# ksadov/FREUD

Measured on AMD Instinct MI355X. Metric: SAE train activations/sec (d=384 dict 8x), higher is better.
Workload: dtype bf16; 1 GPU; Whisper-tiny d=384 dict 8x (n=3072) L1 SAE train step, M=65536 rows/GPU/step, RAdam+cosine, x bfloat16 resident in HBM (BASELINE configs[1]); rows_per_gpu=65536, d_model=384, n_dict=3072, parallelism=dp1, dp=none

## Files before the change

freud_amd/csrc/engine.hip:

```cpp
#include <hip/hip_runtime.h>
#include <math.h>
#include <stdarg.h>
#include <stdio.h>
#include <string.h>

#include <algorithm>
#include <utility>
#include <vector>

#include "../../include/freud_sae.h"
#include "l1_kernels.h"
#include "gemm256.h"
#include "gemm256s.h"
#include "gemm256_fp8.h"
#include "l1_fp8.h"
#include "dp_kernels.h"
#include "p2p_exchange.h"
#include <rccl/rccl.h>
#include <mutex>
#include <unistd.h>

static thread_local bool g_force_gemm128 = false;
static thread_local bool g_no_stream = false;
static thread_local int g_device = 0;
// ... 1398 lines not shown
  g2.nbm = g.nbm / 2;
  g2.nbn = g.nbn / 2;
  hipLaunchKernelGGL(kerns, dim3(G2_PERSIST_STATIC), dim3(512), G2S_LDS_BYTES, s, g2, epi);
  HIP_TRY(hipGetLastError());
  return SAE_OK;
}

template <int AM, int BM_, class Epi>
static int launch_gemm(const GemmArgs& g, const Epi& epi, hipStream_t s) {
  if constexpr (epi_stream<Epi>::value && AM == OP_ROW && BM_ == OP_ROW) {
    if (gemm_streams<AM, BM_, Epi>(g)) return launch_gemm_stream(g, epi, s);
  }
  if (!g_force_gemm128 && g.nbm % 2 == 0 && g.nbn % 2 == 0) {
    auto kern256 = gemm256_bf16_kernel<AM, BM_, Epi>;
    constexpr bool a3 = epi_deep_a_ring<Epi>::value;
    constexpr int lds256 = a3 ? G2_A3_LDS_BYTES : (epi_rounds_first<Epi>::value && G2_BF16_LDS_BYTES > G2_LDS_BYTES) ? G2_BF16_LDS_BYTES : G2_LDS_BYTES;
    static_assert(G2_A3_LDS_BYTES >= G2_BF16_LDS_BYTES && G2_A3_LDS_BYTES >= G2_LDS_BYTES, "the epilogues reuse the ring's LDS");
    LDS_ATTR(kern256, lds256, g_device);
    GemmArgs g2 = g;
    g2.nbm = g.nbm / 2;
    g2.nbn = g.nbn / 2;
    const int grid_max = (g.dyn && g.grid_cover > 0) ? g.grid_cover
                         : g2.tail_tiles > 0    ? g2.nbm * g2.nbn + g2.tail_tiles * (g2.tail_pieces - 1)
                                                : g2.nbm * g2.nbn * g2.splits;
    const int grid_est = (((g.grid_hint + 3) / 4 + 7) / 8) * 8;
    if (G2_PERSIST_STATIC > 0 && !g.dyn && g2.splits == 1 && g2.tail_tiles == 0 && grid_max >= 4 * G2_PERSIST_STATIC) {
      auto kernp = gemm256_bf16_kernel<AM, BM_, Epi, true>;
      LDS_ATTR(kernp, lds256, g_device);
      hipLaunchKernelGGL(kernp, dim3(G2_PERSIST_STATIC), dim3(512), lds256, s, g2, epi);
    } else if (g.dyn && g.grid_hint > 0 && grid_est < grid_max) {
      auto kernp = gemm256_bf16_kernel<AM, BM_, Epi, true>;
      LDS_ATTR(kernp, lds256, g_device);
      hipLaunchKernelGGL(kernp, dim3(grid_est < 256 ? 256 : grid_est), dim3(512), lds256, s, g2, epi);
    } else {
      hipLaunchKernelGGL(kern256, dim3(grid_max), dim3(512), lds256, s, g2, epi);
    }
    HIP_TRY(hipGetLastError());
    return SAE_OK;
  }
  auto kern = gemm_bf16_kernel<AM, BM_, Epi>;
  LDS_ATTR(kern, GEMM_LDS_BYTES, g_device);
  const int grid = (g.dyn && g.grid_cover > 0) ? g.grid_cover : g.nbm * g.nbn * g.splits;
  hipLaunchKernelGGL(kern, dim3(grid), dim3(256), GEMM_LDS_BYTES, s, g, epi);
  HIP_TRY(hipGetLastError());
  return SAE_OK;
}

template <class Epi>
static bool gemm8_streams(const Gemm8Args& g) {
  if constexpr (!epi_stream<Epi>::value) return false;
  return !g_no_stream && g.ktiles >= 2 && g.lda == g.ldb && g.nbm * g.nbn >= 4 * G2_PERSIST_STATIC;
}

template <class Epi>
static int launch_gemm8(const Gemm8Args& g, const Epi& epi, hipStream_t s) {
  if constexpr (epi_stream<Epi>::value) {
    if (gemm8_streams<Epi>(g)) {
      auto kerns = gemm256s_fp8_kernel<Epi>;
      LDS_ATTR(kerns, G2S_LDS_BYTES, g_device);
      hipLaunchKernelGGL(kerns, dim3(G2_PERSIST_STATIC), dim3(512), G2S_LDS_BYTES, s, g, epi);
      HIP_TRY(hipGetLastError());
      return SAE_OK;
    }
  }
  auto kern = gemm256_fp8_kernel<Epi>;
  constexpr int lds = g8_lds_bytes<Epi>();
  LDS_ATTR(kern, lds, g_device);
  hipLaunchKernelGGL(kern, dim3(g.nbm * g.nbn), dim3(512), lds, s, g, epi);
  HIP_TRY(hipGetLastError());
  return SAE_OK;
}

static void prep_weights_l1(sae_ctx* c, hipStream_t s) {
  const int d_p = c->d_p, n_p = c->n_p;
  float* W = c->P;
  if (c->wn_pending && !c->wn_fwd_seen) {
    c->wn_fwd_seen = true;
  } else {
    settle_weights(c, s);
    if (!c->cn_valid) hipLaunchKernelGGL(colnorm_partial_kernel, dim3(n_p / 128, d_p / 32), dim3(256), 0, s, W, c->cn_part, n_p);
    c->cn_valid = false;
    hipLaunchKernelGGL(normalize_cast_kernel, dim3(n_p / 64, d_p / 64), dim3(256), 0, s, W, c->cn_part, d_p / 32, c->Wb,
                       c->Wt, d_p, n_p);
  }
}

template <typename T>
static int launch_prep_x(sae_ctx* c, const T* x, int64_t M, int64_t Mp, hipStream_t s) {
  const int d = c->d, d_p = c->d_p;
  const int grid = grid_for(Mp * (d_p / 8), 2048);
  if (d % 8 == 0 && (reinterpret_cast<uintptr_t>(x) & 15) == 0)
    hipLaunchKernelGGL((prep_x_kernel<T, true>), dim3(grid), dim3(256), 0, s, x, c->xb, c->masked, M, d, Mp, d_p);
  else
    hipLaunchKernelGGL((prep_x_kernel<T, false>), dim3(grid), dim3(256), 0, s, x, c->xb, c->masked, M, d, Mp, d_p);
  return grid;
}

static GemmArgs enc_gemm_args(const sae_ctx* c, const bf16_t* xb, int64_t Mp) {
  GemmArgs g{};
  g.A0 = xb; g.B0 = c->Wt; g.lda = c->d_p; g.ldb = c->d_p;
  g.nbm = (int)(Mp / 128); g.nbn = c->n_p / 128; g.ktiles0 = g.ktiles = c->d_p / 64; g.splits = 1;
  return g;
}

template <typename T>
static auto launch_encoder(sae_ctx* c, const GemmArgs& g, int64_t M, hipStream_t s) {
  EpiEnc e{};
  e.c = c->c; e.bias = c->P + c->nW; e.l1_part = c->l1_part; e.M = M; e.n_p = c->n_p; e.nbn = g.nbn;
  if (gemm_streams<OP_ROW, OP_ROW, EpiEnc>(g)) HIP_TRY(hipMemsetAsync(c->l1_part, 0, (size_t)g.nbm * g.nbn * 4, s));
  ev_begin(c, KID_ENC_FWD, s);
  const int rc = launch_gemm<OP_ROW, OP_ROW>(g, e, s);
  ev_end(c, KID_ENC_FWD, s);
  return rc;
}

template <typename T> static constexpr bool x_dtype_is_bf16() { return false; }
template <> constexpr bool x_dtype_is_bf16<bf16_t>() { return true; }

template <typename T>
static int forward_impl(sae_ctx* c, const T* x, int64_t M, int64_t Mp, hipStream_t s, bool need_backward) {
  const int d = c->d, d_p = c->d_p, n_p = c->n_p;
  const float alpha = (float)c->cfg.recon_alpha;
  float* W = c->P;
  float* b = c->P + c->nW;

  ev_begin(c, KID_PREP_W, s);
  prep_weights_l1(c, s);
  if (c->fp8) hipLaunchKernelGGL(fp8_cast_w_kernel, dim3(n_p / 64, d_p / 64), dim3(256), 0, s, W, c->W8, c->W8t, d_p, n_p);
  ev_end(c, KID_PREP_W, s);

  ev_begin(c, KID_PREP_X, s);
  const bool alias_x = c->use_fused_fwd && sizeof(T) == 2 && x_dtype_is_bf16<T>() && d == d_p && M == Mp &&
                       (reinterpret_cast<uintptr_t>(x) & 15) == 0;
  c->xb_cur = alias_x ? reinterpret_cast<const bf16_t*>(x) : c->xb;
  if (!alias_x) {
    const int grid = launch_prep_x(c, x, M, Mp, s);
    if (!c->use_fused_fwd) {
      const double* gs = (need_backward && c->dp_world > 0) ? c->stats : nullptr;
      if (gs && c->dist) HIP_TRY(hipStreamWaitEvent(s, c->ev_stats, 0));
      hipLaunchKernelGGL(finalize_count_kernel, dim3(1), dim3(256), 0, s, c->masked, grid, c->scal, M, d, alpha, gs);
    }
  }
  if (c->fp8) {
    const int sgrid = (int)((Mp / 4) < 1024 ? (Mp / 4) : 1024);
    hipLaunchKernelGGL(fp8_x_stats_kernel, dim3(sgrid), dim3(256), 0, s, c->xb, Mp, d_p, c->x8_part);
    hipLaunchKernelGGL(fp8_scales_kernel, dim3(1), dim3(256), 0, s, c->x8_part, sgrid, b, c->n, c->scal8);
    const int64_t n8 = Mp * (d_p / 8);
    hipLaunchKernelGGL(fp8_quant_x_kernel, dim3(grid_for(n8, 2048)), dim3(256), 0, s, c->xb, c->x8, n8, c->scal8);
  }
  ev_end(c, KID_PREP_X, s);

  int rc;
  if (c->use_fused_fwd) {
    const int lds = FF_LDS_BYTES;
    FwdFusedArgs a{};
    a.xb = c->xb_cur; a.x = x; a.Wt = c->Wt; a.bias = b; a.cnt_part = c->cnt_part; a.c = c->c; a.dxh = c->dxh;
    a.l1_part = c->l1_part; a.sq_part = c->sq_part; a.M = M; a.d = d; a.n_p = n_p; a.ntiles = n_p / FF_BN;
    a.c_rows = c->max_rows_p;
    const int full_wgs = (int)(M / FF_BM), all_wgs = (int)(Mp / FF_BM);
    auto launch = [&](auto kern, int blocks, int block_offset) -> int {
      LDS_ATTR(kern, 160 * 1024, g_device);
      a.block_offset = block_offset;
      hipLaunchKernelGGL(kern, dim3(blocks), dim3(256), lds, s, a);
      return SAE_OK;
    };
    ev_begin(c, KID_FWD_FUSED, s);
    int rcl = SAE_OK;
    if (full_wgs > 0 && c->cfg.debug_flags == 65 && c->fwd_variant == 1) {
      a.stamps = reinterpret_cast<unsigned long long*>(c->dpre);
      rcl = launch(fwd_fused_d384_kernel<T, false, true>, full_wgs, 0);
    } else if (c->fwd_variant == 2) {
      if (full_wgs > 0 && c->cfg.debug_flags == 65) {
        a.stamps = reinterpret_cast<unsigned long long*>(c->dpre);
        rcl = launch(fwd_fused2_d384_kernel<T, false, true>, full_wgs, 0);
      } else if (full_wgs > 0) rcl = launch(fwd_fused2_d384_kernel<T, false>, full_wgs, 0);
      if (!rcl && all_wgs > full_wgs) rcl = launch(fwd_fused2_d384_kernel<T, true>, all_wgs - full_wgs, full_wgs);
      if (rcl) return rcl;
      ev_end(c, KID_FWD_FUSED, s);
      HIP_TRY(hipGetLastError());
      return SAE_OK;
    } else if (full_wgs > 0) {
      rcl = launch(fwd_fused_d384_kernel<T, false, false>, full_wgs, 0);
    }
    if (!rcl && all_wgs > full_wgs) rcl = launch(fwd_fused_d384_kernel<T, true, false>, all_wgs - full_wgs, full_wgs);
    if (rcl) return rcl;
    ev_end(c, KID_FWD_FUSED, s);
    HIP_TRY(hipGetLastError());
    return SAE_OK;
  }
  if (c->fp8) {
    {
      Gemm8Args g{};
      g.A = c->x8; g.B = c->W8t; g.lda = d_p; g.ldb = d_p;
      g.nbm = (int)(Mp / 256); g.nbn = n_p / 256; g.ktiles = d_p / 128;
      EpiEnc8 e{};
      e.c = c->c; e.c8 = c->c8; e.bias = b; e.scal8 = c->scal8; e.l1_part = c->l1_part; e.M = M; e.n_p = n_p; e.nbn = n_p / 128;
      if (gemm8_streams<EpiEnc8>(g)) HIP_TRY(hipMemsetAsync(c->l1_part, 0, (size_t)(Mp / 128) * (n_p / 128) * 4, s));
      ev_begin(c, KID_ENC_FWD, s);
      rc = launch_gemm8(g, e, s);
      ev_end(c, KID_ENC_FWD, s);
      if (rc) return rc;
    }
    {
      Gemm8Args g{};
      g.A = c->c8; g.B = c->W8; g.lda = n_p; g.ldb = n_p;
      g.nbm = (int)(Mp / 256); g.nbn = d_p / 256; g.ktiles = n_p / 128;
      EpiDec<T> e{};
      e.x = x; e.dxh = c->dxh; e.scal = c->scal; e.sq_part = c->sq_part; e.M = M; e.d = d; e.d_p = d_p; e.nbn = d_p / 128;
      e.vec_all = (M == Mp && d == d_p && d % 4 == 0 && (reinterpret_cast<uintptr_t>(x) % (4 * sizeof(T))) == 0) ? 1 : 0;
      e.vscale = c->scal8 + S8_INV_DEC;
      ev_begin(c, KID_DEC_FWD, s);
      rc = launch_gemm8(g, e, s);
      ev_end(c, KID_DEC_FWD, s);
      if (rc) return rc;
    }
    if (need_backward && c->dxhT) {
      hipLaunchKernelGGL(transpose_bf16_kernel, dim3((unsigned)(Mp / 64), d_p / 64), dim3(256), 0, s, c->dxh, c->dxhT, Mp, d_p);
      hipLaunchKernelGGL(transpose_bf16_kernel, dim3((unsigned)(Mp / 64), d_p / 64), dim3(256), 0, s, c->xb_cur, c->xT, Mp, d_p);
      HIP_TRY(hipGetLastError());
    }
    return SAE_OK;
  }
  rc = launch_encoder<T>(c, enc_gemm_args(c, c->xb_cur, Mp), M, s);
  if (rc) return rc;
  {
    GemmArgs g{};
    g.A0 = c->c; g.B0 = c->Wb; g.lda = n_p; g.ldb = n_p;
    g.nbm = (int)(Mp / 128); g.nbn = d_p / 128; g.ktiles0 = g.ktiles = n_p / 64; g.splits = 1;
    g.group_m = 4;
    EpiDec<T> e{};
    e.x = x; e.dxh = c->dxh; e.scal = c->scal; e.sq_part = c->sq_part; e.M = M; e.d = d; e.d_p = d_p; e.nbn = g.nbn;
    e.vec_all = (M == Mp && d == d_p && d % 4 == 0 && (reinterpret_cast<uintptr_t>(x) % (4 * sizeof(T))) == 0) ? 1 : 0;
    ev_begin(c, KID_DEC_FWD, s);
    rc = launch_gemm<OP_ROW, OP_ROW>(g, e, s);
    ev_end(c, KID_DEC_FWD, s);
    if (rc) return rc;
  }
  if (need_backward && c->dxhT) {
    hipLaunchKernelGGL(transpose_bf16_kernel, dim3((unsigned)(Mp / 64), d_p / 64), dim3(256), 0, s, c->dxh, c->dxhT, Mp, d_p);
    hipLaunchKernelGGL(transpose_bf16_kernel, dim3((unsigned)(Mp / 64), d_p / 64), dim3(256), 0, s, c->xb_cur, c->xT, Mp, d_p);
    HIP_TRY(hipGetLastError());
  }
  return SAE_OK;
}

template <typename T>
static int fwd_bwd_impl(sae_ctx* c, const T* x, int64_t M, hipStream_t s, bool backward) {
  const int d = c->d, d_p = c->d_p, n_p = c->n_p;
  const int64_t Mp = round_up(M, c->row_pad);
  const float alpha = (float)c->cfg.recon_alpha;
  const double* gs = (backward && c->dp_world > 0) ? c->stats : nullptr;
  ev_begin(c, KID_STEP_TOTAL, s);
  int rc = forward_impl<T>(c, x, M, Mp, s, backward);
  if (rc) return rc;
  const bool fold_finalize = c->use_fused_fwd && c->use_fused_bwd && backward && gs == nullptr && c->bwd_ranges == 1 &&
                             c->cfg.debug_flags != 78;
  if (c->use_fused_fwd && !fold_finalize) {
    StatsPush push{};
    if (gs && inline_stats(c)) {
      for (int r = 0; r < c->dp_world; ++r) push.inbox[r] = c->p2p_sig[r] + P2P_SIG_WORDS;
      push.rank = c->p2p_rank; push.world = c->dp_world; push.epoch = ++c->p2p_epoch_push;
      push.timeout_ticks = c->p2p_timeout_ticks; push.status = c->p2p_status; push.status_host = c->p2p_status_hostdev; push.gstats_out = c->stats;
    } else if (gs && c->dist) {
      HIP_TRY(hipStreamWaitEvent(s, c->ev_stats, 0));
    }
    if (push.world > 0) ev_begin(c, KID_STATS_XCHG, s);
    hipLaunchKernelGGL(finalize_losses_kernel, dim3(1), dim3(1024), 0, s, c->l1_part, (int)(Mp / 128), c->sq_part,
                       (int)(Mp / 128), c->scal, c->G + c->nparams, M, d, alpha, c->cnt_part, (int)(Mp / 128),
                       push.world > 0 ? (const double*)nullptr : gs, push);
    if (push.world > 0) ev_end(c, KID_STATS_XCHG, s);
  }
  bool dw_chunked_any = false;
  if (backward) {
    int splits = c->dw_splits;
    int db_rows = (int)(Mp / 128);
    bool dw_chunked = false;
    if (c->use_fused_bwd) {
      BwdFusedArgs a{};
      a.dxh = c->dxh; a.xb = c->xb_cur; a.c = c->c; a.Wt = c->Wt; a.scal = c->scal; a.slab = c->slab; a.db_part = c->db_part;
      a.unscaled = c->use_fused_fwd ? 1 : 0;
      if (fold_finalize) { a.cnt_part = c->cnt_part; a.n_cnt = (int)(Mp / 128); a.alpha = alpha; a.M = M; a.d = d; }
      a.n_p = n_p; a.steps_total = (int)(Mp / BF_BM);
      a.clk = c->cfg.debug_flags == 66 ? reinterpret_cast<unsigned long long*>(c->dpre) + (1 << 16) : nullptr;
      const int nranges = c->bwd_ranges, rtiles = (n_p / BF_BN) / nranges;
      splits = nranges == 1 ? c->bwd_splits : c->bwd_range_splits;
      if (splits > a.steps_total) splits = a.steps_total;
      a.ntiles = rtiles; a.splits = splits;
      db_rows = splits;
      const bool balanced = nranges == 1 && c->bal_m > 0 && a.steps_total >= 64;
      if (balanced) {
        a.bal_m = c->bal_m;
        a.bal_q = (a.steps_total + 31) / 32;
        a.wg_map = c->bal_map;
      }
      const bool dp_now = c->dist && c->dp_world > 0;
      bf16_t* gb = (dp_now && c->payload == SAE_DTYPE_BF16) ? c->Gb : (bf16_t*)nullptr;
      ev_begin(c, KID_BWD_FUSED, s);
      LDS_ATTR(bwd_fused_d384_kernel, BF_LDS_BYTES, g_device);
      for (int r = 0; r < nranges; ++r) {
        a.tile0 = r * rtiles;
        hipLaunchKernelGGL(bwd_fused_d384_kernel, dim3(balanced ? c->bal_grid : a.ntiles * a.splits), dim3(256), BF_LDS_BYTES, s, a);
        if (nranges > 1) {
          const int c0 = a.tile0 * BF_BN, cols = rtiles * BF_BN;
          hipLaunchKernelGGL(reduce_grads_range_kernel, dim3(256), dim3(256), 0, s, c->slab, c->nW, splits, c->db_part, db_rows, n_p,
                             d_p, c0, cols, c->G, c->gn_part + 256 * r, gb);
          if (dp_now && r + 1 < nranges) fused_exchange(c, r, nranges, c0, cols, false, s);
        }
      }
      ev_end(c, KID_BWD_FUSED, s);
      HIP_TRY(hipGetLastError());
    } else {
      if (c->fp8_bwd) {
        const int sgrid = (int)((Mp / 4) < 1024 ? (Mp / 4) : 1024);
        hipLaunchKernelGGL(fp8_x_stats_kernel, dim3(sgrid), dim3(256), 0, s, c->dxh, Mp, d_p, c->x8_part);
        hipLaunchKernelGGL(fp8_g_scale_kernel, dim3(1), dim3(256), 0, s, c->x8_part, sgrid, c->scal8);
        const int64_t n8 = Mp * (d_p / 8);
        hipLaunchKernelGGL(fp8_quant_x_kernel, dim3(grid_for(n8, 2048)), dim3(256), 0, s, c->dxh, c->dxh8, n8, c->scal8, (int)S8_SG);
        Gemm8Args g{};
        g.A = c->dxh8; g.B = c->W8t; g.lda = d_p; g.ldb = d_p;
        g.nbm = (int)(Mp / 256); g.nbn = n_p / 256; g.ktiles = d_p / 128;
        EpiDpre8 e{};
        e.c = c->c; e.dpre = c->dpre; e.db_part = c->db_part; e.scal = c->scal; e.scal8 = c->scal8; e.n_p = n_p;
        ev_begin(c, KID_DPRE, s);
        rc = launch_gemm8(g, e, s);
        ev_end(c, KID_DPRE, s);
// ... 1426 lines not shown
```

freud_amd/csrc/fwd_fused2.h:

```cpp
#pragma once
#include "fwd_fused.h"

typedef __attribute__((ext_vector_type(2))) float f32x2_t;

template <typename T, bool PAD, bool STAMP = false>
__global__ __launch_bounds__(256, 1) void fwd_fused2_d384_kernel(FwdFusedArgs a) {
  extern __shared__ __attribute__((aligned(16))) char smem[];
  const int t = threadIdx.x, lane = t & 63, w = t >> 6;
  const int arow = lane & 31, ah = lane >> 5;
  const int wg = blockIdx.x + a.block_offset;
  const int64_t m0 = (int64_t)wg * FF_BM + 32 * w;
  const int64_t mrow = m0 + arow;
  const bool row_ok = mrow < a.M;
  char* cst = smem + FF_RING_BYTES;
  float* bias_s = reinterpret_cast<float*>(smem + FF_FIXED_LDS);
  unsigned long long clk_k0 = 0, clk_t0 = 0, clk_r0 = 0, clk_t1 = 0;
  if (STAMP) clk_k0 = __builtin_amdgcn_s_memtime();

  typedef __attribute__((ext_vector_type(2))) unsigned short us2_t;
  constexpr unsigned MASK_BITS2 = std::is_same<T, bf16_t>::value ? 0xBF80BF80u : 0xBC00BC00u;
  constexpr bool SCAN_EARLY = !PAD && std::is_same<T, bf16_t>::value;
  bool wany_early = false;

  bf16x8 xfrag[24];
  unsigned voff_t[6], loff_t[6];
#pragma unroll
  for (int i = 0; i < 6; ++i) {
    const int inst = w + 4 * i, sub = inst >> 3, row = 4 * (inst & 7) + (lane >> 4), pc = lane & 15;
    const int ch = pc ^ (((row & 3) << 2) | ((row >> 2) & 3));
    voff_t[i] = (unsigned)(row * (FF_D * 2) + (sub * 16 + ch) * 16);
    loff_t[i] = (unsigned)__builtin_amdgcn_readfirstlane(sub * 8192 + (inst & 7) * 1024);
  }
  typedef __attribute__((address_space(3))) char* lptr_t;
  const unsigned smem_base = (unsigned)(uintptr_t)(lptr_t)smem;
  auto dma_pair = [&](int p, int jt, int st) {
    const bf16_t* src = a.Wt + (int64_t)jt * FF_BN * FF_D;
    const unsigned dst = smem_base + st * FF_WT_BYTES;
    glds16_x2(src, src, voff_t[2 * p], voff_t[2 * p + 1], (unsigned)__builtin_amdgcn_readfirstlane((int)(dst + loff_t[2 * p])),
              (unsigned)__builtin_amdgcn_readfirstlane((int)(dst + loff_t[2 * p + 1])));
  };
  auto dma_one = [&](int k, int jt, int st) {
    const bf16_t* src = a.Wt + (int64_t)jt * FF_BN * FF_D;
    glds16(src, voff_t[k], (unsigned)__builtin_amdgcn_readfirstlane((int)(smem_base + st * FF_WT_BYTES + loff_t[k])));
  };
  const int last = a.ntiles - 1;
#pragma unroll
  for (int q = 0; q < 3; ++q)
#pragma unroll
    for (int p = 0; p < 3; ++p) dma_pair(p, q <= last ? q : last, q);
  static_assert(2 * FF_BN == 64, "one 4-byte piece per lane of wave 0");
  if (w == 0) glds4(a.bias, (unsigned)(lane * 4), (unsigned)__builtin_amdgcn_readfirstlane((int)(smem_base + FF_FIXED_LDS)));
  {
    const bf16_t* xp = a.xb + mrow * FF_D + 8 * ah;
#pragma unroll
    for (int kk = 0; kk < 24; ++kk) xfrag[kk] = *reinterpret_cast<const bf16x8*>(xp + 16 * kk);
  }
  for (int i = t; i < FF_WT_BYTES / 16; i += 256) reinterpret_cast<u32x4*>(smem + 3 * FF_WT_BYTES)[i] = u32x4{0u, 0u, 0u, 0u};
  for (int i = t; i < FF_CST_BYTES / 16; i += 256) reinterpret_cast<u32x4*>(cst)[i] = u32x4{0u, 0u, 0u, 0u};

  f32x16 acc[12];
#pragma unroll
  for (int i = 0; i < 12; ++i)
#pragma unroll
    for (int r = 0; r < 16; ++r) acc[i][r] = 0.f;

  if (SCAN_EARLY) {
    us2_t mz = {0xFFFFu, 0xFFFFu};
#pragma unroll
    for (int kk = 0; kk < 24; ++kk) {
      const u32x4 xw = __builtin_bit_cast(u32x4, xfrag[kk]);
#pragma unroll
      for (int c = 0; c < 4; ++c) mz = __builtin_elementwise_min(mz, __builtin_bit_cast(us2_t, xw[c] ^ MASK_BITS2));
    }
    wany_early = __builtin_amdgcn_ballot_w64((mz[0] == 0) | (mz[1] == 0)) != 0ull;
  }
#pragma unroll
  for (int kk = 0; kk < 24; ++kk) asm volatile("" : "+v"(xfrag[kk]));
  asm volatile("s_waitcnt vmcnt(0)" ::: "memory");
  __syncthreads();

  int roff[8];
#pragma unroll
  for (int i = 0; i < 8; ++i) roff[i] = dual_off(arow, 2 * i + ah);
  int aoff0[6], aoff1[6];
  {
    const int g = (lane >> 4) & 1, q = (lane & 15) >> 2, p = lane & 3;
#pragma unroll
    for (int f = 0; f < 6; ++f) {
      const int ks = f / 3, dt = 3 * w + f % 3;
      const int col = 32 * (dt & 3) + 16 * g + 4 * p;
      const int r0 = 4 * ah + q, r1 = r0 + 8;
      const int base = (dt >> 2) * 8192 + ks * 4096;
      aoff0[f] = base + dual_off(r0, col >> 3) + (col & 7) * 2;
      aoff1[f] = base + dual_off(r1, col >> 3) + (col & 7) * 2;
    }
  }
  typedef __attribute__((ext_vector_type(8))) short s16x8;
  auto tr_pair = [&](const char* p0, const char* p1) -> bf16x8 {
    const s16x4 lo = __builtin_amdgcn_ds_read_tr16_b64_v4i16(LDS_PTR(s16x4, p0));
    const s16x4 hi = __builtin_amdgcn_ds_read_tr16_b64_v4i16(LDS_PTR(s16x4, p1));
    const s16x8 v = __builtin_shufflevector(lo, hi, 0, 1, 2, 3, 4, 5, 6, 7);
    return __builtin_bit_cast(bf16x8, v);
  };
  auto swz = [](int row) { return (row & 7) ^ ((row >> 1) & 1) ^ ((row >> 4) & 1); };
  int boff[4];
#pragma unroll
  for (int i = 0; i < 4; ++i) boff[i] = arow * 128 + (((4 * (i >> 1) + 2 * (i & 1) + ah) ^ swz(arow)) << 4);
  const int wrow = w * 4096;
  const int drow_l = lane >> 3, dch = lane & 7;
  int doff0, doff1;
  {
    const int tl = dch >> 2, s = (dch & 3) >> 1, u = dch & 1;
    doff0 = drow_l * 128 + (((4 * tl + 2 * s + 0) ^ swz(drow_l)) << 4) + 8 * u;
    doff1 = drow_l * 128 + (((4 * tl + 2 * s + 1) ^ swz(drow_l)) << 4) + 8 * u;
  }
  auto dpiece = [](int off, int p) { return (p & 2) ? (off ^ 16) : off; };
  bf16_t* cdrain = a.c + (m0 + drow_l) * a.n_p + dch * 8;

  float l1_acc = 0.f;

  f32x16 Sn;
#pragma unroll
  for (int r = 0; r < 16; ++r) Sn[r] = 0.f;
#pragma unroll
  for (int kk = 0; kk < 24; ++kk) {
    const bf16x8 fa = *reinterpret_cast<const bf16x8*>(smem + (kk >> 3) * 8192 + roff[kk & 7]);
    Sn = __builtin_amdgcn_mfma_f32_32x32x16_bf16(fa, xfrag[kk], Sn, 0, 0, 0);
  }

  constexpr int RING = 8;
  const char *rlo[8], *rhi[8];
#pragma unroll
  for (int i = 0; i < 8; ++i) {
    rlo[i] = smem + roff[i];
    rhi[i] = smem + 2 * FF_WT_BYTES + roff[i];
  }
  const char *a0lo[6], *a1lo[6], *a0hi[6], *a1hi[6];
#pragma unroll
  for (int f = 0; f < 6; ++f) {
    a0lo[f] = smem + aoff0[f];
    a1lo[f] = smem + aoff1[f];
    a0hi[f] = smem + 2 * FF_WT_BYTES + aoff0[f];
    a1hi[f] = smem + 2 * FF_WT_BYTES + aoff1[f];
  }
  const char* bptr[4];
#pragma unroll
  for (int i = 0; i < 4; ++i) bptr[i] = cst + boff[i];
  auto dec_a = [&](int slot, int f) -> bf16x8 {
    const int off = (slot & 1) * FF_WT_BYTES;
    return tr_pair((slot < 2 ? a0lo : a0hi)[f] + off, (slot < 2 ? a1lo : a1hi)[f] + off);
  };
  auto enc_frag = [&](int slot, int kk) -> bf16x8 {
    const int off = (slot & 1) * FF_WT_BYTES + (kk >> 3) * 8192;
    return *reinterpret_cast<const bf16x8*>((slot < 2 ? rlo : rhi)[kk & 7] + off);
  };
  auto dec_b = [&](int pb, int hf, int b) -> bf16x8 {
    const int ks = b >> 2, mb = b & 3;
    return *reinterpret_cast<const bf16x8*>(bptr[2 * hf + ks] + pb * 16384 + mb * 4096);
  };

  bf16x8 ring[RING], Afr[6], Bq[4];
  f32x16 SA = Sn, SB;
#pragma unroll
  for (int r = 0; r < 16; ++r) SB[r] = 0.f;
#pragma unroll
  for (int f = 0; f < 3; ++f) Afr[f] = dec_a(3, f);
  Bq[0] = dec_b(1, 1, 0);
  Bq[1] = dec_b(1, 1, 1);
#pragma unroll
  for (int k = 0; k < 3; ++k) ring[k] = enc_frag(1, k);

#ifdef FF2_WAITSTAMP
  unsigned long long ws_vm = 0, ws_bar = 0, ws_gap = 0, ws_prev = 0;
#endif
  u32x4 dr[2];
  bf16_t* const dummy_line = a.c + (int64_t)a.c_rows * a.n_p + lane * 8;
  auto body = [&](auto ph_tag, int j) {
    constexpr int PH = decltype(ph_tag)::value;
    constexpr int SLOT_D = (PH + 3) & 3, SLOT_DN = PH, SLOT_E = (PH + 1) & 3, SLOT_EN = (PH + 2) & 3, SLOT_DMA = (PH + 3) & 3;
    constexpr int PB_W = (PH >> 1) & 1, HF_W = PH & 1;
    constexpr int PB_D = (((PH + 3) & 3) >> 1) & 1, HF_D = (PH + 3) & 1;
    f32x16& Scur = (PH & 1) ? SB : SA;
    f32x16& Snxt = (PH & 1) ? SA : SB;
    const int jt = j + 3 <= last ? j + 3 : last;
    const float* bj = bias_s + (j & (FF_BIAS_RING_TILES - 1)) * FF_BN;
    const char* cst_r = cst + (PB_W ^ 1) * 16384 + wrow;
    bf16_t* dst_pair = j >= 2 ? cdrain + 64 * ((j >> 1) - 1) : dummy_line;
    const int64_t dst_rstride = j >= 2 ? (int64_t)a.n_p : 0;
    f32x4 bq[4];
    float l1_it = 0.f;
    unsigned se_u = 0u;
    float se_t0 = 0.f, se_t1 = 0.f;
    bf16x8 cw;
    const f32x16 S = Scur;

    static_for<0, 48>([&](auto slot_tag) {
      constexpr int i = decltype(slot_tag)::value;
      if ((i & 3) == 0 && i <= 40) {
        if (i / 2 + 4 <= 23) ring[(i / 2 + 4) % RING] = enc_frag(SLOT_E, i / 2 + 4);
        ring[(i / 2 + 3) % RING] = enc_frag(SLOT_E, i / 2 + 3);
      }
      if (i == 42 || i == 44 || i == 46) ring[(i - 42) / 2] = enc_frag(SLOT_EN, (i - 42) / 2);
      if (i == 15 || i == 16 || i == 17) Afr[i - 12] = dec_a(SLOT_D, i - 12);
      if (i == 45 || i == 46 || i == 47) Afr[i - 45] = dec_a(SLOT_DN, i - 45);
      if (i >= 5 && i <= 35 && (i - 5) % 6 == 0) Bq[((i + 7) / 6) & 3] = dec_b(PB_D, HF_D, (i + 7) / 6);
      if (i == 41) Bq[0] = dec_b(PB_W, HF_W, 0);
      if (i == 47) Bq[1] = dec_b(PB_W, HF_W, 1);
      if (i < 4) bq[i] = *reinterpret_cast<const f32x4*>(bj + 8 * i + 4 * ah);
      if (i == 40) {
        __builtin_amdgcn_sched_barrier(0);
#ifdef FF2_WAITSTAMP
        const unsigned long long w0 = __builtin_amdgcn_s_memtime();
        asm volatile("s_waitcnt vmcnt(1) lgkmcnt(0)" ::: "memory");
        const unsigned long long w1 = __builtin_amdgcn_s_memtime();
        asm volatile("s_waitcnt lgkmcnt(0)" ::: "memory");
        __builtin_amdgcn_s_barrier();
        const unsigned long long w2 = __builtin_amdgcn_s_memtime();
        ws_vm += w1 - w0; ws_bar += w2 - w1;
        if (ws_prev != 0) ws_gap += w0 - ws_prev;
        ws_prev = w2;
#else
        asm volatile("s_waitcnt vmcnt(1) lgkmcnt(2)" ::: "memory");
        __builtin_amdgcn_s_barrier();
#endif
        __builtin_amdgcn_sched_barrier(0);
      }
      if (i == 41 || i == 45) dma_one((i - 41) / 4, jt, SLOT_DMA);
      if (i == 1 || i == 5 || i == 9 || i == 13) dma_one(2 + (i - 1) / 4, j + 2 <= last ? j + 2 : last, (PH + 2) & 3);
      if ((PH & 1) == 0 && i == 46 && w == 0) {
        const int jb = j + 2 <= a.ntiles - 2 ? j + 2 : a.ntiles - 2;
        glds4(a.bias + (int64_t)jb * FF_BN, (unsigned)(lane * 4),
              (unsigned)__builtin_amdgcn_readfirstlane((int)(smem_base + FF_FIXED_LDS + ((j + 2) & (FF_BIAS_RING_TILES - 1)) * FF_BN * 4)));
      }
      if (i >= 4 && i <= 35) {
        const int p = (i - 4) >> 2, ph = (i - 4) & 3, e0 = 2 * p;
        if (ph == 0) {
          se_u = __builtin_bit_cast(unsigned, __builtin_convertvector(f32x2_t{S[e0], S[e0 + 1]}, bf16x2));
        } else if (ph == 1) {
          se_t0 = __uint_as_float(se_u << 16) + bq[e0 >> 2][e0 & 3];
          se_t1 = __uint_as_float(se_u & 0xFFFF0000u);
        } else if (ph == 2) {
          se_t1 = se_t1 + bq[e0 >> 2][(e0 & 3) + 1];
          se_t0 = fmaxf(se_t0, 0.f);
          se_t1 = fmaxf(se_t1, 0.f);
          if (PAD) { se_t0 = row_ok ? se_t0 : 0.f; se_t1 = row_ok ? se_t1 : 0.f; }
        } else {
          asm volatile("v_add_f32 %0, %0, %1\n\tv_add_f32 %0, %0, %2" : "+v"(l1_it) : "v"(se_t0), "v"(se_t1));
          cw[e0 & 7] = (bf16_t)se_t0;
          cw[(e0 & 7) + 1] = (bf16_t)se_t1;
          if ((e0 & 7) == 6)
            *reinterpret_cast<bf16x8*>(cst + PB_W * 16384 + wrow + boff[2 * HF_W + (e0 >> 3)]) = cw;
        }
      }
      if (i == 29 || i == 33) {
        const int p = 2 * (PH & 1) + (i == 33);
        const uint2 lo = *reinterpret_cast<const uint2*>(cst_r + p * 1024 + dpiece(doff0, p));
        const uint2 hi = *reinterpret_cast<const uint2*>(cst_r + p * 1024 + dpiece(doff1, p));
        dr[i == 33] = u32x4{lo.x, lo.y, hi.x, hi.y};
      }
      if (i == 37 || i == 42) {
        const int p = 2 * (PH & 1) + (i == 42);
        __builtin_nontemporal_store(dr[i == 42], reinterpret_cast<u32x4*>(dst_pair + (int64_t)(8 * p) * dst_rstride));
      }
      __builtin_amdgcn_sched_barrier(0);
      if ((i & 1) == 0) {
        const int m = i / 2, ks = m / 12, mb = (m % 12) / 3, dtl = m % 3;
        acc[4 * dtl + mb] = __builtin_amdgcn_mfma_f32_32x32x16_bf16(Afr[3 * ks + dtl], Bq[(4 * ks + mb) & 3], acc[4 * dtl + mb], 0, 0, 0);
      } else if (i == 1) {
        f32x16 zero;
#pragma unroll
        for (int r = 0; r < 16; ++r) zero[r] = 0.f;
        Snxt = __builtin_amdgcn_mfma_f32_32x32x16_bf16(ring[0], xfrag[0], zero, 0, 0, 0);
      } else {
        Snxt = __builtin_amdgcn_mfma_f32_32x32x16_bf16(ring[(i / 2) % RING], xfrag[i / 2], Snxt, 0, 0, 0);
      }
      __builtin_amdgcn_sched_barrier(0);
    });
    l1_acc += l1_it + 0.0f;
  };
  if (STAMP) { clk_t0 = __builtin_amdgcn_s_memtime(); clk_r0 = __builtin_amdgcn_s_memrealtime(); }
  for (int j4 = 0; j4 < a.ntiles; j4 += 4) {
    body(std::integral_constant<int, 0>{}, j4);
    body(std::integral_constant<int, 1>{}, j4 + 1);
    body(std::integral_constant<int, 2>{}, j4 + 2);
    body(std::integral_constant<int, 3>{}, j4 + 3);
  }
  if (STAMP) {
    const unsigned long long t1 = __builtin_amdgcn_s_memtime(), r1 = __builtin_amdgcn_s_memrealtime();
    clk_t1 = t1;
    if (lane == 0) {
      unsigned long long* o = a.stamps + ((int64_t)wg * 4 + w) * 8;
      o[0] = o[1] = o[2] = 0; o[3] = (unsigned long long)a.ntiles; o[4] = t1 - clk_t0; o[5] = r1 - clk_r0; o[6] = clk_t0 - clk_k0;
    }
  }
  Bq[2] = dec_b(1, 1, 2);
#pragma unroll
  for (int m = 0; m < 24; ++m) {
    if (m == 3 || m == 4 || m == 5) Afr[m] = dec_a(3, m);
    if (m % 3 == 0 && m / 3 + 3 <= 7) Bq[(m / 3 + 3) & 3] = dec_b(1, 1, m / 3 + 3);
    __builtin_amdgcn_sched_barrier(0);
    const int ks = m / 12, mb = (m % 12) / 3, dtl = m % 3;
    acc[4 * dtl + mb] = __builtin_amdgcn_mfma_f32_32x32x16_bf16(Afr[3 * ks + dtl], Bq[(4 * ks + mb) & 3], acc[4 * dtl + mb], 0, 0, 0);
    __builtin_amdgcn_sched_barrier(0);
  }
  {
    const char* cst_r = cst + (((a.ntiles >> 1) - 1) & 1) * 16384 + wrow;
#pragma unroll
    for (int p = 0; p < 4; ++p) {
      const uint2 lo = *reinterpret_cast<const uint2*>(cst_r + p * 1024 + dpiece(doff0, p));
      const uint2 hi = *reinterpret_cast<const uint2*>(cst_r + p * 1024 + dpiece(doff1, p));
      __builtin_nontemporal_store(u32x4{lo.x, lo.y, hi.x, hi.y},
                                  reinterpret_cast<u32x4*>(cdrain + (int64_t)(8 * p) * a.n_p + 64 * ((a.ntiles >> 1) - 1)));
    }
  }
  __builtin_amdgcn_sched_barrier(0);
  asm volatile("s_waitcnt vmcnt(4) lgkmcnt(0)" ::: "memory");
  __builtin_amdgcn_s_barrier();
  __builtin_amdgcn_sched_barrier(0);

  unsigned long long clk_e0 = 0, clk_e1 = 0, clk_e2 = 0;
  if (STAMP) clk_e0 = __builtin_amdgcn_s_memtime();
  float sq = 0.f, plain = 0.f, nmask = 0.f;
  float msq = 0.f;
  f32x2_t plain2 = {0.f, 0.f};
  typedef __attribute__((ext_vector_type(4))) T Tx4;
  const bool vec_ok = (a.d == FF_D) && ((reinterpret_cast<uintptr_t>(a.x) & (sizeof(T) * 4 - 1)) == 0);
  constexpr int FF_DXH_PITCH = FF_D * 2 + 16;
  static_assert(128 * FF_DXH_PITCH <= FF_FIXED_LDS, "the dx_hat staging must fit the idle LDS");
  char* stg = smem;
  constexpr bool X_VIA_LDS = !PAD && sizeof(T) == 2;
  constexpr bool X_FROM_FRAGS = X_VIA_LDS && std::is_same<T, bf16_t>::value;
  unsigned* mflag = reinterpret_cast<unsigned*>(smem + FF_FIXED_LDS + 64);
  bool blk_masked = true;
  if (X_FROM_FRAGS && vec_ok && reinterpret_cast<const void*>(a.x) == reinterpret_cast<const void*>(a.xb)) {
    char* srow_w = stg + (32 * w + arow) * FF_DXH_PITCH + 16 * ah;
    us2_t mz = {0xFFFFu, 0xFFFFu};
#pragma unroll
    for (int kk = 0; kk < 24; ++kk) {
      *reinterpret_cast<bf16x8*>(srow_w + 32 * kk) = xfrag[kk];
      if (!SCAN_EARLY) {
        const u32x4 xw = __builtin_bit_cast(u32x4, xfrag[kk]);
#pragma unroll
        for (int c = 0; c < 4; ++c) mz = __builtin_elementwise_min(mz, __builtin_bit_cast(us2_t, xw[c] ^ MASK_BITS2));
      }
    }
    const bool wany = SCAN_EARLY ? wany_early : __builtin_amdgcn_ballot_w64((mz[0] == 0) | (mz[1] == 0)) != 0ull;
    if (lane == 0) mflag[w] = wany ? 1u : 0u;
    __syncthreads();
    const u32x4 f = *reinterpret_cast<const u32x4*>(mflag);
    blk_masked = (f[0] | f[1] | f[2] | f[3]) != 0u;
  } else
  if (X_VIA_LDS && vec_ok) {
    const char* xblk = reinterpret_cast<const char*>(reinterpret_cast<const T*>(a.x) + m0 * FF_D);
    us2_t mz = {0xFFFFu, 0xFFFFu};
#pragma unroll
    for (int p0 = 0; p0 < 24; p0 += 4) {
      u32x4 xr[4];
#pragma unroll
      for (int pc = 0; pc < 4; ++pc) xr[pc] = *reinterpret_cast<const u32x4*>(xblk + (p0 + pc) * 1024 + lane * 16);
#pragma unroll
      for (int pc = 0; pc < 4; ++pc) {
        const int off = (p0 + pc) * 1024 + lane * 16, r = off / (FF_D * 2), cb = off - r * (FF_D * 2);
        *reinterpret_cast<u32x4*>(stg + (32 * w + r) * FF_DXH_PITCH + cb) = xr[pc];
#pragma unroll
        for (int c = 0; c < 4; ++c) mz = __builtin_elementwise_min(mz, __builtin_bit_cast(us2_t, xr[pc][c] ^ MASK_BITS2));
      }
    }
    const bool wany = __builtin_amdgcn_ballot_w64((mz[0] == 0) | (mz[1] == 0)) != 0ull;
    if (lane == 0) mflag[w] = wany ? 1u : 0u;
    __syncthreads();
    const u32x4 f = *reinterpret_cast<const u32x4*>(mflag);
    blk_masked = (f[0] | f[1] | f[2] | f[3]) != 0u;
  }
  if (STAMP) clk_e1 = __builtin_amdgcn_s_memtime();
  auto residual = [&](auto notest_tag) {
  constexpr bool NOTEST = decltype(notest_tag)::value;
  constexpr bool FENCE = NOTEST && X_VIA_LDS;
  constexpr bool PIPE = FENCE && std::is_same<T, bf16_t>::value;
  Tx4 xq[2][4];
  auto xload = [&](int g, Tx4 (&dst)[4]) {
    const char* sr = stg + (32 * (g / 3) + arow) * FF_DXH_PITCH + (96 * w + 32 * (g % 3) + 4 * ah) * 2;
#pragma unroll
    for (int k = 0; k < 4; ++k) dst[k] = *reinterpret_cast<const Tx4*>(sr + 16 * k);
  };
  if constexpr (PIPE) xload(0, xq[0]);
#pragma unroll
  for (int mb = 0; mb < 4; ++mb) {
    const int64_t grow = (int64_t)wg * FF_BM + 32 * mb + arow;
    const bool ok = !PAD || grow < a.M;
    const float rmask = ok ? 1.f : 0.f;
    const T* xrow = reinterpret_cast<const T*>(a.x) + (ok ? grow : a.M - 1) * a.d;
    char* srow = stg + (32 * mb + arow) * FF_DXH_PITCH;
#pragma unroll
    for (int dtl = 0; dtl < 3; ++dtl) {
      const int dbase = 96 * w + 32 * dtl + 4 * ah;
      if (NOTEST || vec_ok) {
        const int g = 3 * mb + dtl;
        if constexpr (FENCE) {
          if (g > 0) __builtin_amdgcn_sched_barrier(0);
          if (PIPE && g + 1 < 12) xload(g + 1, xq[(g + 1) & 1]);
        }
        Tx4 xv[4];
#pragma unroll
        for (int k = 0; k < 4; ++k)
          xv[k] = PIPE ? xq[g & 1][k]
                       : (X_VIA_LDS ? *reinterpret_cast<const Tx4*>(srow + (dbase + 8 * k) * 2) : *reinterpret_cast<const Tx4*>(xrow + dbase + 8 * k));
        if (!PAD) {
          if constexpr (NOTEST && X_VIA_LDS) {
            if constexpr (std::is_same<T, bf16_t>::value) {
              uint2 ow[4];
#pragma unroll
              for (int k = 0; k < 4; ++k) {
                const uint2 xw = __builtin_bit_cast(uint2, xv[k]);
#pragma unroll
                for (int pp = 0; pp < 2; ++pp) {
                  const unsigned xd = pp ? xw.y : xw.x;
                  const unsigned rb = __builtin_bit_cast(unsigned, __builtin_convertvector(
                      f32x2_t{acc[4 * dtl + mb][4 * k + 2 * pp], acc[4 * dtl + mb][4 * k + 2 * pp + 1]}, bf16x2));
                  const f32x2_t rf = {__uint_as_float(rb << 16), __uint_as_float(rb & 0xFFFF0000u)};
                  const f32x2_t xf = {__uint_as_float(xd << 16), __uint_as_float(xd & 0xFFFF0000u)};
                  f32x2_t e2, d2;
                  asm("v_pk_add_f32 %0, %1, %2 neg_lo:[0,1] neg_hi:[0,1]" : "=v"(e2) : "v"(rf), "v"(xf));
                  asm("v_pk_fma_f32 %0, %1, %1, %0" : "+v"(plain2) : "v"(e2));
                  asm("v_pk_add_f32 %0, %1, %1" : "=v"(d2) : "v"(e2));
                  const unsigned ob = __builtin_bit_cast(unsigned, __builtin_convertvector(d2, bf16x2));
                  if (pp) ow[k].y = ob; else ow[k].x = ob;
                }
              }
#pragma unroll
              for (int k = 0; k < 4; ++k) *reinterpret_cast<uint2*>(srow + (dbase + 8 * k) * 2) = ow[k];
              continue;
            }
            bf16x4 o[4];
#pragma unroll
            for (int k = 0; k < 4; ++k)
#pragma unroll
              for (int q = 0; q < 4; ++q) {
                const float xf = (float)xv[k][q];
                const float e = bf16_round(acc[4 * dtl + mb][4 * k + q]) - xf;
                plain = __builtin_fmaf(e, e, plain);
                o[k][q] = (bf16_t)(e + e);
              }
#pragma unroll
            for (int k = 0; k < 4; ++k) *reinterpret_cast<bf16x4*>(srow + (dbase + 8 * k) * 2) = o[k];
            continue;
          }
          bf16x4 o[4];
          unsigned nm_i = 0u;
#pragma unroll
          for (int k = 0; k < 4; ++k)
#pragma unroll
            for (int q = 0; q < 4; ++q) {
              const float xf = (float)xv[k][q];
              const float e = bf16_round(acc[4 * dtl + mb][4 * k + q]) - xf;
              const bool mk = xf == -1.0f;
              const float em = mk ? e : 0.0f, ek = mk ? 0.0f : e;
              plain = __builtin_fmaf(e, e, plain);
              msq = __builtin_fmaf(em, em, msq);
              nm_i += mk ? 1u : 0u;
              o[k][q] = (bf16_t)(ek + ek);
            }
          nmask += (float)nm_i;
#pragma unroll
          for (int k = 0; k < 4; ++k) *reinterpret_cast<bf16x4*>(srow + (dbase + 8 * k) * 2) = o[k];
          continue;
        }
#pragma unroll
        for (int k = 0; k < 4; ++k) {
          bf16x4 o;
#pragma unroll
          for (int q = 0; q < 4; ++q) {
            const float xf = (float)xv[k][q];
            const float e = bf16_round(acc[4 * dtl + mb][4 * k + q]) - xf;
            const float e2 = e * e;
            plain += rmask * e2;
            const float keep = (xf != -1.0f) ? rmask : 0.f;
            nmask += rmask - keep;
            sq += keep * e2;
            o[q] = (bf16_t)(keep * (e * 2.0f));
          }
          *reinterpret_cast<bf16x4*>(srow + (dbase + 8 * k) * 2) = o;
        }
      } else {
#pragma unroll
        for (int k = 0; k < 4; ++k) {
          bf16x4 o;
#pragma unroll
          for (int q = 0; q < 4; ++q) {
            const int dd = dbase + 8 * k + q;
            const bool valid = dd < a.d;
            const float xf = (float)xrow[valid ? dd : a.d - 1];
            const float e = bf16_round(acc[4 * dtl + mb][4 * k + q]) - xf;
            const float e2 = valid ? e * e : 0.f;
            plain += rmask * e2;
            const float keep = (valid && xf != -1.0f) ? rmask : 0.f;
            nmask += (valid ? rmask : 0.f) - keep;
            sq += keep * e2;
            o[q] = (bf16_t)(keep * (e * 2.0f));
          }
          *reinterpret_cast<bf16x4*>(srow + (dbase + 8 * k) * 2) = o;
        }
      }
    }
  }
  };
  if (X_VIA_LDS && vec_ok && !blk_masked) residual(std::true_type{}); else residual(std::false_type{});
  if (STAMP) clk_e2 = __builtin_amdgcn_s_memtime();
  __syncthreads();
  {
    char* gblk = reinterpret_cast<char*>(a.dxh + m0 * FF_D);
#pragma unroll
    for (int pc = 0; pc < 24; ++pc) {
      const int off = pc * 1024 + lane * 16, r = off / (FF_D * 2), cb = off - r * (FF_D * 2);
      *reinterpret_cast<u32x4*>(gblk + off) = *reinterpret_cast<const u32x4*>(stg + (32 * w + r) * FF_DXH_PITCH + cb);
    }
  }
  plain += plain2[0] + plain2[1];
  if (!PAD && vec_ok) sq = plain - msq;
  float* red = reinterpret_cast<float*>(smem + FF_FIXED_LDS);
  {
    const float v0 = wave_sum(l1_acc), v1 = wave_sum(sq), v2 = wave_sum(plain), v3 = wave_sum(nmask);
    if (lane == 0) *reinterpret_cast<f32x4*>(red + 4 * w) = f32x4{v0, v1, v2, v3};
  }
  lds_barrier();
  const float l1s = ((red[0] + red[4]) + red[8]) + red[12];
  const float sqs = ((red[1] + red[5]) + red[9]) + red[13];
  const float pls = ((red[2] + red[6]) + red[10]) + red[14];
  const float nms = ((red[3] + red[7]) + red[11]) + red[15];
  if (STAMP && lane == 0) {
    unsigned long long* o = a.stamps + ((int64_t)wg * 4 + w) * 8;
    const unsigned long long te = __builtin_amdgcn_s_memtime();
    o[7] = te - clk_k0;
    o[0] = clk_e0 - clk_t1; o[1] = clk_e1 - clk_e0; o[2] = clk_e2 - clk_e1;
#ifdef FF2_WAITSTAMP
    o[0] = ws_vm; o[1] = ws_bar; o[2] = ws_gap;
#endif
  }
  if (t == 0) {
    a.cnt_part[wg] = nms;
    a.l1_part[wg] = l1s;
    a.sq_part[2 * wg] = sqs;
    a.sq_part[2 * wg + 1] = pls;
  }
}
```

Before: 112.8 million activations/s.

## Make fused forward kernel persistent, overlapping next block's loads with residual epilogue

Adds a persistent variant of the fused forward d384 kernel. It launches one workgroup per CU and loops over row blocks. During the residual epilogue of the current block it prefetches the next block's weight tiles, bias and x fragments. The epilogue is split into four 32-row quarters staged through two LDS buffers, with global stores per quarter. This aims to hide per-block prologue latency and launch tail effects, at the cost of extra LDS, more barriers and more complex control flow.

Measured after the change: 112.9 million activations/s, median of 2. Within noise of the previous version (+0.1%).

```diff
diff --git a/freud_amd/csrc/engine.hip b/freud_amd/csrc/engine.hip
--- a/freud_amd/csrc/engine.hip
+++ b/freud_amd/csrc/engine.hip
@@ -1574,16 +1574,15 @@
 
   int rc;
   if (c->use_fused_fwd) {
-    const int lds = FF_LDS_BYTES;
     FwdFusedArgs a{};
     a.xb = c->xb_cur; a.x = x; a.Wt = c->Wt; a.bias = b; a.cnt_part = c->cnt_part; a.c = c->c; a.dxh = c->dxh;
     a.l1_part = c->l1_part; a.sq_part = c->sq_part; a.M = M; a.d = d; a.n_p = n_p; a.ntiles = n_p / FF_BN;
     a.c_rows = c->max_rows_p;
     const int full_wgs = (int)(M / FF_BM), all_wgs = (int)(Mp / FF_BM);
-    auto launch = [&](auto kern, int blocks, int block_offset) -> int {
+    auto launch = [&](auto kern, int blocks, int block_offset, int lds_bytes = FF_LDS_BYTES) -> int {
       LDS_ATTR(kern, 160 * 1024, g_device);
       a.block_offset = block_offset;
-      hipLaunchKernelGGL(kern, dim3(blocks), dim3(256), lds, s, a);
+      hipLaunchKernelGGL(kern, dim3(blocks), dim3(256), lds_bytes, s, a);
       return SAE_OK;
     };
     ev_begin(c, KID_FWD_FUSED, s);
@@ -1592,7 +1591,19 @@
       a.stamps = reinterpret_cast<unsigned long long*>(c->dpre);
       rcl = launch(fwd_fused_d384_kernel<T, false, true>, full_wgs, 0);
     } else if (c->fwd_variant == 2) {
-      if (full_wgs > 0 && c->cfg.debug_flags == 65) {
+      bool persistent = false;
+      if constexpr (x_dtype_is_bf16<T>()) persistent = d == FF_D && c->cfg.debug_flags != 87;
+      if (full_wgs > 0 && persistent) {
+        if constexpr (x_dtype_is_bf16<T>()) {
+          static thread_local int cus = 0;
+          if (cus <= 0) HIP_TRY(hipDeviceGetAttribute(&cus, hipDeviceAttributeMultiprocessorCount, g_device));
+          const int grid = c->cfg.debug_flags == 88 ? 1 : (full_wgs < cus ? full_wgs : cus);
+          if (c->cfg.debug_flags == 65) {
+            a.stamps = reinterpret_cast<unsigned long long*>(c->dpre);
+            rcl = launch(fwd_fused2p_d384_kernel<true>, grid, 0, FF2P_LDS_BYTES);
+          } else rcl = launch(fwd_fused2p_d384_kernel<false>, grid, 0, FF2P_LDS_BYTES);
+        }
+      } else if (full_wgs > 0 && c->cfg.debug_flags == 65) {
         a.stamps = reinterpret_cast<unsigned long long*>(c->dpre);
         rcl = launch(fwd_fused2_d384_kernel<T, false, true>, full_wgs, 0);
       } else if (full_wgs > 0) rcl = launch(fwd_fused2_d384_kernel<T, false>, full_wgs, 0);
diff --git a/freud_amd/csrc/fwd_fused2.h b/freud_amd/csrc/fwd_fused2.h
--- a/freud_amd/csrc/fwd_fused2.h
+++ b/freud_amd/csrc/fwd_fused2.h
@@ -3,13 +3,19 @@
 
 typedef __attribute__((ext_vector_type(2))) float f32x2_t;
 
-template <typename T, bool PAD, bool STAMP = false>
-__global__ __launch_bounds__(256, 1) void fwd_fused2_d384_kernel(FwdFusedArgs a) {
+constexpr int FF2_DXH_PITCH = FF_D * 2 + 16;
+constexpr int FF2_QUARTER_BYTES = 32 * FF2_DXH_PITCH;
+constexpr int FF2P_LDS_BYTES = FF_LDS_BYTES + FF2_QUARTER_BYTES + 128;
+static_assert(FF2P_LDS_BYTES <= 160 * 1024 && FF2_QUARTER_BYTES <= FF_CST_BYTES, "the quarters must fit the LDS of a CU");
+
+template <typename T, bool PAD, bool STAMP, bool PERSIST>
+__device__ __forceinline__ void fwd_fused2_d384_body(const FwdFusedArgs& a) {
+  static_assert(!PERSIST || (!PAD && std::is_same<T, bf16_t>::value), "the persistent form walks full blocks of bf16 activations");
   extern __shared__ __attribute__((aligned(16))) char smem[];
   const int t = threadIdx.x, lane = t & 63, w = t >> 6;
   const int arow = lane & 31, ah = lane >> 5;
-  const int wg = blockIdx.x + a.block_offset;
-  const int64_t m0 = (int64_t)wg * FF_BM + 32 * w;
+  int wg = blockIdx.x + a.block_offset;
+  int64_t m0 = (int64_t)wg * FF_BM + 32 * w;
   const int64_t mrow = m0 + arow;
   const bool row_ok = mrow < a.M;
   char* cst = smem + FF_RING_BYTES;
@@ -44,20 +50,32 @@
     glds16(src, voff_t[k], (unsigned)__builtin_amdgcn_readfirstlane((int)(smem_base + st * FF_WT_BYTES + loff_t[k])));
   };
   const int last = a.ntiles - 1;
+  auto prologue_w = [&](int tid) {
 #pragma unroll
   for (int q = 0; q < 3; ++q)
 #pragma unroll
     for (int p = 0; p < 3; ++p) dma_pair(p, q <= last ? q : last, q);
   static_assert(2 * FF_BN == 64, "one 4-byte piece per lane of wave 0");
-  if (w == 0) glds4(a.bias, (unsigned)(lane * 4), (unsigned)__builtin_amdgcn_readfirstlane((int)(smem_base + FF_FIXED_LDS)));
-  {
-    const bf16_t* xp = a.xb + mrow * FF_D + 8 * ah;
+  if ((tid >> 6) == 0) glds4(a.bias, (unsigned)((tid & 63) * 4), (unsigned)__builtin_amdgcn_readfirstlane((int)(smem_base + FF_FIXED_LDS)));
+  };
+  auto load_x = [&](int64_t row, int h) {
+    const bf16_t* xp = a.xb + row * FF_D + 8 * h;
 #pragma unroll
     for (int kk = 0; kk < 24; ++kk) xfrag[kk] = *reinterpret_cast<const bf16x8*>(xp + 16 * kk);
-  }
-  for (int i = t; i < FF_WT_BYTES / 16; i += 256) reinterpret_cast<u32x4*>(smem + 3 * FF_WT_BYTES)[i] = u32x4{0u, 0u, 0u, 0u};
-  for (int i = t; i < FF_CST_BYTES / 16; i += 256) reinterpret_cast<u32x4*>(cst)[i] = u32x4{0u, 0u, 0u, 0u};
-
+  };
+  auto zero_slot3 = [&](int tid) {
+  for (int i = tid; i < FF_WT_BYTES / 16; i += 256) reinterpret_cast<u32x4*>(smem + 3 * FF_WT_BYTES)[i] = u32x4{0u, 0u, 0u, 0u};
+  };
+  auto zero_cst = [&](int tid) {
+  for (int i = tid; i < FF_CST_BYTES / 16; i += 256) reinterpret_cast<u32x4*>(cst)[i] = u32x4{0u, 0u, 0u, 0u};
+  };
+  prologue_w(t);
+  load_x(mrow, ah);
+  zero_slot3(t);
+  zero_cst(t);
+
+  bool has_next = false;
+  do {
   f32x16 acc[12];
 #pragma unroll
   for (int i = 0; i < 12; ++i)
@@ -313,6 +331,12 @@
                                   reinterpret_cast<u32x4*>(cdrain + (int64_t)(8 * p) * a.n_p + 64 * ((a.ntiles >> 1) - 1)));
     }
   }
+  unsigned* pflag = reinterpret_cast<unsigned*>(smem + FF_LDS_BYTES + FF2_QUARTER_BYTES);
+  int te = t, zero_e = 0;
+  if constexpr (PERSIST) {
+    asm volatile("" : "+v"(te), "+v"(zero_e));
+    if ((te & 63) == 0) pflag[te >> 6] = wany_early ? 1u : 0u;
+  }
   __builtin_amdgcn_sched_barrier(0);
   asm volatile("s_waitcnt vmcnt(4) lgkmcnt(0)" ::: "memory");
   __builtin_amdgcn_s_barrier();
@@ -324,15 +348,15 @@
   float msq = 0.f;
   f32x2_t plain2 = {0.f, 0.f};
   typedef __attribute__((ext_vector_type(4))) T Tx4;
-  const bool vec_ok = (a.d == FF_D) && ((reinterpret_cast<uintptr_t>(a.x) & (sizeof(T) * 4 - 1)) == 0);
-  constexpr int FF_DXH_PITCH = FF_D * 2 + 16;
+  const bool vec_ok = PERSIST || ((a.d == FF_D) && ((reinterpret_cast<uintptr_t>(a.x) & (sizeof(T) * 4 - 1)) == 0));
+  constexpr int FF_DXH_PITCH = FF2_DXH_PITCH;
   static_assert(128 * FF_DXH_PITCH <= FF_FIXED_LDS, "the dx_hat staging must fit the idle LDS");
   char* stg = smem;
   constexpr bool X_VIA_LDS = !PAD && sizeof(T) == 2;
   constexpr bool X_FROM_FRAGS = X_VIA_LDS && std::is_same<T, bf16_t>::value;
   unsigned* mflag = reinterpret_cast<unsigned*>(smem + FF_FIXED_LDS + 64);
   bool blk_masked = true;
-  if (X_FROM_FRAGS && vec_ok && reinterpret_cast<const void*>(a.x) == reinterpret_cast<const void*>(a.xb)) {
+  if (!PERSIST && X_FROM_FRAGS && vec_ok && reinterpret_cast<const void*>(a.x) == reinterpret_cast<const void*>(a.xb)) {
     char* srow_w = stg + (32 * w + arow) * FF_DXH_PITCH + 16 * ah;
     us2_t mz = {0xFFFFu, 0xFFFFu};
 #pragma unroll
@@ -350,7 +374,7 @@
     const u32x4 f = *reinterpret_cast<const u32x4*>(mflag);
     blk_masked = (f[0] | f[1] | f[2] | f[3]) != 0u;
   } else
-  if (X_VIA_LDS && vec_ok) {
+  if (!PERSIST && X_VIA_LDS && vec_ok) {
     const char* xblk = reinterpret_cast<const char*>(reinterpret_cast<const T*>(a.x) + m0 * FF_D);
     us2_t mz = {0xFFFFu, 0xFFFFu};
 #pragma unroll
@@ -373,32 +397,33 @@
     blk_masked = (f[0] | f[1] | f[2] | f[3]) != 0u;
   }
   if (STAMP) clk_e1 = __builtin_amdgcn_s_memtime();
-  auto residual = [&](auto notest_tag) {
+  auto residual = [&](auto notest_tag, auto mb_lo_tag, auto mb_hi_tag, char* rows) {
   constexpr bool NOTEST = decltype(notest_tag)::value;
+  constexpr int MB_LO = decltype(mb_lo_tag)::value, MB_HI = decltype(mb_hi_tag)::value;
   constexpr bool FENCE = NOTEST && X_VIA_LDS;
   constexpr bool PIPE = FENCE && std::is_same<T, bf16_t>::value;
   Tx4 xq[2][4];
   auto xload = [&](int g, Tx4 (&dst)[4]) {
-    const char* sr = stg + (32 * (g / 3) + arow) * FF_DXH_PITCH + (96 * w + 32 * (g % 3) + 4 * ah) * 2;
+    const char* sr = rows + (32 * (g / 3 - MB_LO) + arow) * FF_DXH_PITCH + (96 * w + 32 * (g % 3) + 4 * ah) * 2;
 #pragma unroll
     for (int k = 0; k < 4; ++k) dst[k] = *reinterpret_cast<const Tx4*>(sr + 16 * k);
   };
-  if constexpr (PIPE) xload(0, xq[0]);
-#pragma unroll
-  for (int mb = 0; mb < 4; ++mb) {
+  if constexpr (PIPE) xload(3 * MB_LO, xq[(3 * MB_LO) & 1]);
+#pragma unroll
+  for (int mb = MB_LO; mb < MB_HI; ++mb) {
     const int64_t grow = (int64_t)wg * FF_BM + 32 * mb + arow;
     const bool ok = !PAD || grow < a.M;
     const float rmask = ok ? 1.f : 0.f;
     const T* xrow = reinterpret_cast<const T*>(a.x) + (ok ? grow : a.M - 1) * a.d;
-    char* srow = stg + (32 * mb + arow) * FF_DXH_PITCH;
+    char* srow = rows + (32 * (mb - MB_LO) + arow) * FF_DXH_PITCH;
 #pragma unroll
     for (int dtl = 0; dtl < 3; ++dtl) {
       const int dbase = 96 * w + 32 * dtl + 4 * ah;
       if (NOTEST || vec_ok) {
         const int g = 3 * mb + dtl;
         if constexpr (FENCE) {
-          if (g > 0) __builtin_amdgcn_sched_barrier(0);
-          if (PIPE && g + 1 < 12) xload(g + 1, xq[(g + 1) & 1]);
+          if (g > 3 * MB_LO) __builtin_amdgcn_sched_barrier(0);
+          if (PIPE && g + 1 < 3 * MB_HI) xload(g + 1, xq[(g + 1) & 1]);
         }
         Tx4 xv[4];
 #pragma unroll
@@ -504,7 +529,45 @@
     }
   }
   };
-  if (X_VIA_LDS && vec_ok && !blk_masked) residual(std::true_type{}); else residual(std::false_type{});
+  typedef std::integral_constant<int, 0> mb0_t;
+  typedef std::integral_constant<int, 4> mb4_t;
+  if constexpr (PERSIST) {
+    const int arow_e = te & 31, ah_e = (te >> 5) & 1;
+    const int wu = __builtin_amdgcn_readfirstlane(te >> 6);
+    const int wg_next = wg + (int)gridDim.x;
+    has_next = wg_next < (int)(a.M / FF_BM);
+    if (has_next) {
+      prologue_w(te);
+      zero_slot3(te);
+    }
+    {
+      const u32x4 f = *reinterpret_cast<const u32x4*>(pflag);
+      blk_masked = (f[0] | f[1] | f[2] | f[3]) != 0u;
+    }
+    static_for<0, 4>([&](auto mb_tag) {
+      constexpr int mb = decltype(mb_tag)::value;
+      char* qb = ((mb & 1) ? smem + FF_LDS_BYTES : cst) + zero_e;
+      if (wu == mb) {
+        char* srow_w = qb + arow_e * FF_DXH_PITCH + 16 * ah_e;
+#pragma unroll
+        for (int kk = 0; kk < 24; ++kk) *reinterpret_cast<bf16x8*>(srow_w + 32 * kk) = xfrag[kk];
+        if (has_next) load_x((int64_t)wg_next * FF_BM + 32 * mb + arow_e, ah_e);
+      }
+      lds_barrier();
+      if (mb == 3 && has_next) zero_cst(te);
+      if (!blk_masked) residual(std::true_type{}, mb_tag, std::integral_constant<int, mb + 1>{}, qb);
+      else residual(std::false_type{}, mb_tag, std::integral_constant<int, mb + 1>{}, qb);
+      lds_barrier();
+      char* gq = reinterpret_cast<char*>(a.dxh + ((int64_t)wg * FF_BM + 32 * mb) * FF_D);
+#pragma unroll
+      for (int pc = 0; pc < 6; ++pc) {
+        const int off = pc * 4096 + te * 16, r = off / (FF_D * 2), cb = off - r * (FF_D * 2);
+        *reinterpret_cast<u32x4*>(gq + off) = *reinterpret_cast<const u32x4*>(qb + r * FF_DXH_PITCH + cb);
+      }
+    });
+    if (STAMP) clk_e1 = clk_e0, clk_e2 = __builtin_amdgcn_s_memtime();
+  } else {
+  if (X_VIA_LDS && vec_ok && !blk_masked) residual(std::true_type{}, mb0_t{}, mb4_t{}, stg); else residual(std::false_type{}, mb0_t{}, mb4_t{}, stg);
   if (STAMP) clk_e2 = __builtin_amdgcn_s_memtime();
   __syncthreads();
   {
@@ -515,22 +578,25 @@
       *reinterpret_cast<u32x4*>(gblk + off) = *reinterpret_cast<const u32x4*>(stg + (32 * w + r) * FF_DXH_PITCH + cb);
     }
   }
+  }
   plain += plain2[0] + plain2[1];
   if (!PAD && vec_ok) sq = plain - msq;
-  float* red = reinterpret_cast<float*>(smem + FF_FIXED_LDS);
+  float* red = reinterpret_cast<float*>(PERSIST ? smem + FF_LDS_BYTES + FF2_QUARTER_BYTES + 64 : smem + FF_FIXED_LDS);
   {
     const float v0 = wave_sum(l1_acc), v1 = wave_sum(sq), v2 = wave_sum(plain), v3 = wave_sum(nmask);
-    if (lane == 0) *reinterpret_cast<f32x4*>(red + 4 * w) = f32x4{v0, v1, v2, v3};
+    if ((te & 63) == 0) *reinterpret_cast<f32x4*>(red + 4 * (te >> 6)) = f32x4{v0, v1, v2, v3};
   }
   lds_barrier();
   const float l1s = ((red[0] + red[4]) + red[8]) + red[12];
   const float sqs = ((red[1] + red[5]) + red[9]) + red[13];
   const float pls = ((red[2] + red[6]) + red[10]) + red[14];
   const float nms = ((red[3] + red[7]) + red[11]) + red[15];
+  unsigned long long clk_end = 0;
+  if (STAMP && PERSIST) clk_end = __builtin_amdgcn_s_memtime();
   if (STAMP && lane == 0) {
     unsigned long long* o = a.stamps + ((int64_t)wg * 4 + w) * 8;
-    const unsigned long long te = __builtin_amdgcn_s_memtime();
-    o[7] = te - clk_k0;
+    const unsigned long long tend = PERSIST ? clk_end : __builtin_amdgcn_s_memtime();
+    o[7] = tend - clk_k0;
     o[0] = clk_e0 - clk_t1; o[1] = clk_e1 - clk_e0; o[2] = clk_e2 - clk_e1;
 #ifdef FF2_WAITSTAMP
     o[0] = ws_vm; o[1] = ws_bar; o[2] = ws_gap;
@@ -542,4 +608,20 @@
     a.sq_part[2 * wg] = sqs;
     a.sq_part[2 * wg + 1] = pls;
   }
+  if constexpr (PERSIST) {
+    wg += (int)gridDim.x;
+    m0 = (int64_t)wg * FF_BM + 32 * w;
+    if (STAMP) clk_k0 = clk_end;
+  }
+  } while (PERSIST && has_next);
 }
+
+template <typename T, bool PAD, bool STAMP = false>
+__global__ __launch_bounds__(256, 1) void fwd_fused2_d384_kernel(FwdFusedArgs a) {
+  fwd_fused2_d384_body<T, PAD, STAMP, false>(a);
+}
+
+template <bool STAMP = false>
+__global__ __launch_bounds__(256, 1) void fwd_fused2p_d384_kernel(FwdFusedArgs a) {
+  fwd_fused2_d384_body<bf16_t, false, STAMP, true>(a);
+}
```
